# daigo0927/pwcnet

Measured on AMD Instinct MI355X. Metric: image_pairs_per_sec_448x1024, higher is better.
Workload: dtype f32 via fp16x2-split MFMA (fp32 tensors and accumulation; big stride-1 convs, level-1 extractor and correlation on the F16 pipe)

## Files before the change

pwcnet_amd/_lib.py:

```python
import ctypes
import os
import subprocess

import torch

_HERE = os.path.dirname(os.path.abspath(__file__))
CSRC = os.path.join(_HERE, "csrc")
HARNESS = os.environ.get("PWC_HARNESS", "") == "1"
LIB_PATH = os.path.join(CSRC, "libpwc_hip_harness.so" if HARNESS else "libpwc_hip.so")
HARNESS_SIGNATURES_NAMES = ("pwc_debug_cost_volume_blk_rows", "pwc_debug_conv3x3_sk_tile", "pwc_debug_conv3x3_t32",
                            "pwc_debug_h2_reserve_cus")
SOURCES = ["conv3x3_mfma.hip", "conv3x3_wino.hip", "conv3x3_direct.hip", "cost_volume.hip", "pwc_ops.hip",
           "pwc_backward.hip", "conv3x3_wgrad.hip", "conv3x3_h2.hip", "conv3x3_c16pair.hip", "conv3x3_sk.hip", "conv3x3_t32.hip", "conv3x3_w32.hip",
           "pwc_flow_loss.hip", "pwc_unsup.hip", "pwc_census.hip", "pwc_fbcheck.hip"]
HEADERS = ["pwc_common.h", "conv_fp32_common.h", "cost_volume_common.h", "loss_common.h", "cost_volume_roll.hip", "cost_volume_mfma.hip", "cost_volume_h2.hip", "cost_volume_blk.hip", "conv3x3_wino4.hip", os.path.join("..", "..", "include", "pwc_hip.h")]

_vp, _i, _f, _l, _sz = ctypes.c_void_p, ctypes.c_int, ctypes.c_float, ctypes.c_long, ctypes.c_size_t

SIGNATURES = {
    "pwc_version": (_i, []),
    "pwc_error_string": (ctypes.c_char_p, [_i]),
    "pwc_cost_volume_f32": (_i, [_vp, _i, _vp, _i, _vp, _i, _i, _i, _i, _i, _i, _f, _vp]),
    "pwc_cost_volume_uses_rolling_kernel": (_i, [_i, _i, _i, _i, _i, _i, _i]),
    "pwc_warp_bilinear_f32": (_i, [_vp, _i, _vp, _i, _f, _vp, _i, _i, _i, _i, _i, _vp]),
    "pwc_warp_nearest_f32": (_i, [_vp, _i, _vp, _i, _f, _vp, _i, _i, _i, _i, _i, _vp]),
    "pwc_cost_volume_coarse_f32": (_i, [_vp, _i, _vp, _i, _vp, _i, _f, _vp, _i, _vp, _i, _i, _i, _i, _i, _i, _f, _vp]),
    "pwc_resize_bilinear_pair_f32": (_i, [_vp, _i, _vp, _i, _vp, _i, _vp, _i, _i, _i, _i, _i, _i, _i, _vp]),
    "pwc_warp_copy_f32": (_i, [_i, _vp, _i, _vp, _i, _f, _vp, _i, _i, _i, _i, _i, _vp, _i, _vp, _i, _i, _vp]),
    "pwc_warp_cost_volume_f32": (_i, [_vp, _i, _vp, _i, _vp, _i, _f, _vp, _i, _i, _i, _i, _i, _i, _f, _vp]),
    "pwc_warp_cost_volume_concat_f32": (_i, [_vp, _i, _vp, _i, _vp, _i, _f, _vp, _i, _i, _vp, _i, _i, _i, _i, _i, _i, _f, _vp]),
    "pwc_warp_cost_volume_concat_h2_f32": (_i, [_vp, _i, _vp, _i, _vp, _i, _f, _vp, _i, _i, _vp, _i, _i, _i, _i, _i, _i, _f, _vp]),
    "pwc_warp_cost_volume_concat_blk_f32": (_i, [_vp, _i, _vp, _i, _vp, _i, _f, _vp, _i, _i, _vp, _i, _i, _i, _i, _i, _i, _f, _vp]),
    "pwc_warp_cost_volume_concat_supported": (_i, [_i, _i, _i, _i, _i, _i, _i, _i, _i]),
    "pwc_warp_cost_volume_concat_blk_supported": (_i, [_i, _i, _i, _i, _i, _i, _i, _i, _i]),
    "pwc_conv3x3_packed_floats": (_sz, [_i, _i]),
    "pwc_conv3x3_pack_f32": (_i, [_vp, _vp, _i, _i, _i, _vp, _vp]),
    "pwc_conv3x3_f32": (_i, [_vp, _i, _vp, _vp, _vp, _i, _i, _i, _i, _i, _i, _i, _i, _i, _f, _i, _i, _vp, _sz, _vp]),
    "pwc_conv3x3_workspace_floats": (_sz, [_i, _i]),
    "pwc_conv3x3_plan": (_i, [_i, _i, _i, ctypes.POINTER(_i)]),
    "pwc_conv3x3_uses_halo_kernel": (_i, [_i, _i, _i, _i, _i]),
    "pwc_conv3x3_tile_shape": (_i, [_i, ctypes.POINTER(_i), ctypes.POINTER(_i)]),
    "pwc_conv3x3_wino_packed_floats": (_sz, [_i, _i]),
    "pwc_conv3x3_wino_pack_f32": (_i, [_vp, _vp, _i, _i, _i, _vp, _vp]),
    "pwc_conv3x3_wino_f32": (_i, [_vp, _i, _vp, _vp, _vp, _i, _i, _i, _i, _i, _i, _i, _i, _f, _vp]),
    "pwc_conv3x3_wino_workgroups": (_l, [_i, _i, _i, _i, _i]),
    "pwc_conv3x3_wino4_packed_floats": (_sz, [_i, _i]),
    "pwc_conv3x3_wino4_pack_f32": (_i, [_vp, _vp, _i, _i, _i, _vp, _vp]),
    "pwc_conv3x3_wino4_f32": (_i, [_vp, _i, _vp, _vp, _vp, _i, _i, _i, _i, _i, _i, _i, _i, _f, _vp]),
    "pwc_conv3x3_wino4_supported": (_i, [_i, _i, _i, _i, _i, _i]),
    "pwc_conv3x3_h2_packed_floats": (_sz, [_i, _i]),
    "pwc_conv3x3_h2_pack_f32": (_i, [_vp, _vp, _i, _i, _i, _vp, _vp]),
    "pwc_conv3x3_h2_f32": (_i, [_vp, _i, _vp, _vp, _vp, _i, _i, _i, _i, _i, _i, _i, _i, _f, _vp, _sz, _vp]),
    "pwc_conv3x3_h2_ex_f32": (_i, [_vp, _i, _i, _vp, _i, _vp, _vp, _vp, _i, _i, _i, _i, _i, _i, _i, _i, _f, _vp, _sz, _vp, _vp]),
    "pwc_conv3x3_h2_ex3_f32": (_i, [_vp, _i, _i, _vp, _i, _i, _vp, _i, _vp, _vp, _vp, _i, _i, _i, _i, _i, _i, _i, _f, _vp, _sz, _vp, _vp]),
    "pwc_conv3x3_h2_workspace_floats": (_sz, [_i, _i, _i, _i, _i, _i]),
    "pwc_conv3x3_h2_supported": (_i, [_i, _i, _i, _i, _i, _i]),
    "pwc_conv3x3_h2_plan": (_i, [_i, _i, _i, _i, _i, _i]),
    "pwc_conv3x3_h2_stride2_f32": (_i, [_vp, _i, _vp, _vp, _vp, _i, _i, _i, _i, _i, _i, _i, _f, _vp, _sz, _vp, _vp]),
    "pwc_conv3x3_h2_stride2_supported": (_i, [_i, _i, _i, _i, _i]),
    "pwc_conv3x3_sk_packed_floats": (_sz, [_i, _i]),
    "pwc_conv3x3_sk_pack_f32": (_i, [_vp, _vp, _i, _i, _i, _vp, _vp]),
    "pwc_conv3x3_sk_f32": (_i, [_vp, _i, _vp, _vp, _vp, _i, _i, _i, _i, _i, _i, _i, _i, _i, _f, _vp]),
    "pwc_conv3x3_sk_supported": (_i, [_i, _i, _i, _i, _i, _i, _i]),
    "pwc_conv3x3_sk_variant_f32": (_i, [_vp, _i, _vp, _vp, _vp, _i, _i, _i, _i, _i, _i, _i, _i, _i, _f, _i, _vp]),
    "pwc_conv3x3_t32_packed_floats": (_sz, [_i]),
    "pwc_conv3x3_t32_pack_f32": (_i, [_vp, _vp, _i, _i, _vp, _vp]),
    "pwc_conv3x3_t32_f32": (_i, [_vp, _i, _vp, _vp, _vp, _i, _i, _i, _i, _i, _i, _i, _i, _f, _vp]),
    "pwc_conv3x3_t32_supported": (_i, [_i, _i, _i, _i, _i, _i]),
    "pwc_conv3x3_w32_packed_floats": (_sz, [_i]),
    "pwc_conv3x3_w32_pack_f32": (_i, [_vp, _vp, _i, _i, _vp, _vp]),
    "pwc_conv3x3_w32_f32": (_i, [_vp, _i, _vp, _vp, _vp, _i, _i, _i, _i, _i, _i, _i, _f, _vp]),
    "pwc_conv3x3_w32_supported": (_i, [_i, _i, _i, _i, _i, _i, _i]),
    "pwc_conv3x3_h2_stride2_packed_floats": (_sz, [_i, _i]),
    "pwc_conv3x3_h2_stride2_pack_f32": (_i, [_vp, _vp, _i, _i, _i, _vp, _vp]),
    "pwc_conv3x3_h2_stride2_workspace_floats": (_sz, [_i, _i, _i, _i, _i]),
    "pwc_conv3x3_c16pair_packed_floats": (_sz, []),
    "pwc_conv3x3_c16pair_pack_f32": (_i, [_vp, _vp, _vp, _vp]),
    "pwc_conv3x3_c16pair_f32": (_i, [_vp, _i, _vp, _vp, _vp, _vp, _i, _i, _i, _i, _f, _vp]),
    "pwc_conv3x3_c16pair_supported": (_i, [_i, _i, _i]),
    "pwc_conv3x3_c3c16pair_packed_floats": (_sz, []),
    "pwc_conv3x3_c3c16pair_pack_f32": (_i, [_vp, _vp, _vp, _vp, _vp]),
    "pwc_conv3x3_c3c16pair_f32": (_i, [_vp, _i, _vp, _i, _vp, _vp, _vp, _vp, _vp, _i, _i, _i, _f, _vp]),
    "pwc_conv3x3_c3c16pair_supported": (_i, [_i, _i, _i]),
    "pwc_conv3x3_h2_variant_f32": (_i, [_vp, _i, _vp, _vp, _vp, _i, _i, _i, _i, _i, _i, _i, _i, _f, _i, _vp, _sz, _vp]),
    "pwc_conv3x3_wino_split_plan": (_i, [_i, _i, _i, _i, _i, _i]),
    "pwc_conv3x3_wino_split_workspace_floats": (_sz, [_i, _i, _i, _i, _i]),
    "pwc_conv3x3_wino_split_f32": (_i, [_vp, _i, _vp, _vp, _vp, _i, _i, _i, _i, _i, _i, _i, _i, _f, _i, _vp, _sz, _vp]),
    "pwc_conv3x3_direct_f32": (_i, [_vp, _i, _vp, _vp, _vp, _i, _vp, _i, _i, _i, _i, _i, _i, _i, _i, _i, _f, _vp]),
    "pwc_resize_bilinear_f32": (_i, [_vp, _i, _vp, _i, _i, _i, _i, _i, _i, _i, _f, _vp]),
    "pwc_resize_bilinear_status_f32": (_i, [_vp, _i, _vp, _i, _i, _i, _i, _i, _i, _i, _f, _vp, _vp]),
    "pwc_absmax_f32": (_i, [_vp, _i, _l, _i, _vp, _vp]),
    "pwc_copy_channels_f32": (_i, [_vp, _i, _vp, _i, _l, _i, _vp]),
    "pwc_device_spin": (_i, [ctypes.c_longlong, _vp]),
    "pwc_device_touch": (_i, [_vp, _vp]),
    "pwc_lrelu_grad_f32": (_i, [_vp, _i, _vp, _i, _l, _i, _f, _vp]),
    "pwc_add_f32": (_i, [_vp, _i, _vp, _i, _l, _i, _f, _i, _vp]),
# ... 123 lines not shown
```

pwcnet_amd/csrc/conv3x3_h2.hip:

```cpp
#pragma once
#include "pwc_common.h"
#include <type_traits>

typedef float pwc_f32x16 __attribute__((ext_vector_type(16)));

struct H2Args {
    const float* x;
    const void* wp;
    const float* bias;
    float* y;
    int x_cs, y_cs;
    int N, H, W;
    int Cin_phys, Cout;
    int apply_act;
    float slope;
    int tiles_x, tiles_y, ncb;
    int dil_y, dil_x;
    int ntiles;
    float* ws_partial;
    unsigned* dbg;
    int Ho, Wo;
    const float* x2;
    int x2_cs, nc16_a;
    const float* x3;
// ... 414 lines not shown
        tap(std::integral_constant<int, 2>{}, std::integral_constant<int, 1>{}, g, buf, more, false);
        H2_STAMP(11);
        tap(std::integral_constant<int, 2>{}, std::integral_constant<int, 2>{}, g, buf, more, false);
        H2_STAMP(12);
        const bool tile_end = c16 == nc16 - 1;
        if (tile_end || !more) {
            if (ABL & 2048) tk0 = __builtin_readcyclecounter();
            if (piece_c0 != 0) {
                finish(tcur, 1, 0);
            } else if (tile_end) {
                finish(tcur, 0, 0);
            } else {
                const long tile_end_g = (long)(g - c16) + nc16;
                int nother = 0;
                for (int w2 = lw + 1; w2 < G && (long)w2 * total / G < tile_end_g; ++w2) ++nother;
                finish(tcur, 0, nother);
            }
            drain = true;
            piece_c0 = 0;
            if (ABL & 2048) tk_fin += __builtin_readcyclecounter() - tk0;
        }
        step(tcur, c16);
        step(t1, c1);
        step(t2, c2);
    }
    if ((ABL & 2048) && a.dbg && lane == 0) {
        unsigned* o = a.dbg + (lw * 8 + wave) * 4;
        o[0] = (unsigned)(__builtin_readcyclecounter() - tk_start); o[1] = (unsigned)tk_wait; o[2] = (unsigned)tk_bar; o[3] = (unsigned)tk_fin;
    }
#undef H2_STAMP
}

__global__ void conv3x3_h2_pack_kernel(const float* __restrict__ w, const int32_t* __restrict__ cin_map, int Cin,
                                       int Cin_phys, int Cout, int nct, unsigned short* __restrict__ packed, int s2) {
    const size_t total = (size_t)(Cin_phys >> 4) * nct * 9 * 32 * 16;
    for (size_t idx = blockIdx.x * (size_t)blockDim.x + threadIdx.x; idx < total;
         idx += (size_t)gridDim.x * blockDim.x) {
        const int ch = (int)(idx & 15);
        size_t r = idx >> 4;
        const int i = (int)(r & 31);
        r >>= 5;
        const int tap = (int)(r % 9);
        r /= 9;
        const int ct = (int)(r % nct);
        const int c16 = (int)(r / nct);
        const int ncc = Cin_phys >> 6, par = s2 ? c16 / ncc : 0;
        const int cphys = s2 ? (c16 - par * ncc) * 16 + ch : c16 * 16 + ch;
        const int clog = cin_map ? cin_map[cphys] : (cphys < Cin ? cphys : -1);
        const int co = ct * 32 + i;
        int wtap = tap;
        if (s2) {
            const int R = tap / 3, DX = tap - 3 * R, dy = 2 * (R - 1) + (par >> 1), dx = 2 * (DX - 1) + (par & 1);
            wtap = (R >= 1 && DX >= 1 && dy <= 2 && dx <= 2) ? dy * 3 + dx : -1;
        }
        float u = 0.f;
        if (wtap >= 0 && clog >= 0 && clog < Cin && co < Cout) u = w[((size_t)wtap * Cin + clog) * Cout + co];
        _Float16 h, m;
        pwc_split1(u, h, m);
        const int tr = tap / 3, dx = tap - 3 * tr;
        unsigned short* base = packed + (((((size_t)c16 * 3 + tr) * nct + ct) * 3 + dx) * 4) * 256;
        base[(ch >> 3) * 256 + i * 8 + (ch & 7)] = __builtin_bit_cast(unsigned short, h);
        base[(2 + (ch >> 3)) * 256 + i * 8 + (ch & 7)] = __builtin_bit_cast(unsigned short, m);
    }
}

extern "C" size_t pwc_conv3x3_h2_packed_floats(int Cin_phys, int Cout) {
    if (Cin_phys <= 0 || Cout <= 0) return 0;
    return (size_t)(Cin_phys >> 4) * ((Cout + 31) / 32) * 9 * (H2_TAPB / 4);
}

extern "C" int pwc_conv3x3_h2_pack_f32(const float* w_hwio, const int32_t* cin_map, int Cin, int Cin_phys,
                                       int Cout, float* packed, pwc_stream_t stream) {
    if (!w_hwio || !packed || Cin <= 0 || Cout <= 0 || Cin_phys < Cin) return PWC_EINVAL;
    if (Cin_phys % 16) return PWC_EALIGN;
    const int nct = (Cout + 31) / 32;
    const size_t total = (size_t)(Cin_phys >> 4) * nct * 9 * 32 * 16;
    int blocks = (int)((total + 255) / 256);
    if (blocks > 4096) blocks = 4096;
    hipLaunchKernelGGL(conv3x3_h2_pack_kernel, dim3(blocks), dim3(256), 0, (hipStream_t)stream, w_hwio, cin_map,
                       Cin, Cin_phys, Cout, nct, reinterpret_cast<unsigned short*>(packed), 0);
    return pwc_launch_status();
}

extern "C" size_t pwc_conv3x3_h2_stride2_packed_floats(int Cin_phys, int Cout) {
    return pwc_conv3x3_h2_packed_floats(4 * Cin_phys, Cout);
}
extern "C" int pwc_conv3x3_h2_stride2_pack_f32(const float* w_hwio, const int32_t* cin_map, int Cin, int Cin_phys,
                                               int Cout, float* packed, pwc_stream_t stream) {
    if (!w_hwio || !packed || Cin <= 0 || Cout <= 0 || Cin_phys < Cin) return PWC_EINVAL;
    if (Cin_phys % 16) return PWC_EALIGN;
    const int nct = (Cout + 31) / 32;
    const size_t total = (size_t)(Cin_phys >> 2) * nct * 9 * 32 * 16;
    int blocks = (int)((total + 255) / 256);
    if (blocks > 4096) blocks = 4096;
    hipLaunchKernelGGL(conv3x3_h2_pack_kernel, dim3(blocks), dim3(256), 0, (hipStream_t)stream, w_hwio, cin_map,
                       Cin, 4 * Cin_phys, Cout, nct, reinterpret_cast<unsigned short*>(packed), 1);
    return pwc_launch_status();
}

struct H2Variant { int couts, rows, nm; };
static inline H2Variant h2_variant(int v) {
    switch (v) {
        case 1: return {128, 8, 12};
        case 2: return {64, 16, 12};
        case 3: return {96, 8, 9};
        case 4: return {32, 16, 6};
        default: return {64, 8, 6};
    }
}
struct H2Geo { int dy, dx, xs, hs, ws; };
static inline H2Geo h2_geometry(int H, int W, int d, int Cout) {
    H2Geo g = {d, d, 1, (H + d - 1) / d, (W + d - 1) / d};
    if (g.ws < 24 && d % 2 == 0 && (W + d / 2 - 1) / (d / 2) >= 24 && Cout % 64 == 0) {
        g.dx = d / 2; g.xs = 2; g.ws = (W + g.dx - 1) / g.dx;
    }
    return g;
}
static inline long h2_blocks(int v, int N, const H2Geo& g, int Cout) {
    const H2Variant t = h2_variant(v);
    return (long)N * g.dy * g.dx * ((g.ws + 31) / 32) * ((g.hs + t.rows - 1) / t.rows) * (Cout / t.couts);
}
static int h2_plan(int N, int H, int W, int Cin_phys, int Cout, int dilation, long* blocks_out) {
    if (N <= 0 || H <= 0 || W <= 0 || dilation < 1 || Cin_phys < 16 || (Cin_phys % 16) || Cout < 32 || (Cout % 32) || Cout > H2_MAX_COUT) return 0;
    const H2Geo geo = h2_geometry(H, W, dilation, Cout);
    int best = 0;
    double best_cost = 0.;
    long best_blocks = 0;
    const int order[5] = {1, 2, 3, 5, 4};
    for (int oi = 0; oi < 5; ++oi) {
        const int v = order[oi];
        const H2Variant t = h2_variant(v);
        if (Cout % t.couts) continue;
        if (geo.xs == 2 && t.rows != 8) continue;
        const long nb = h2_blocks(v, N, geo, Cout);
        if (nb >= (1L << 31)) continue;
        const double cost = (nb <= 256 ? 1.0 : (double)nb / 256.0) * (t.nm + 3.6);
        if (!best || cost < best_cost) { best = v; best_cost = cost; best_blocks = nb; }
    }
    if (blocks_out) *blocks_out = best_blocks;
    return best;
}

static inline bool h2_split_pays(long ntiles, int nc16, int cus) {
    if (ntiles > cus) return ntiles * nc16 >= (long)H2_MIN_STAGES * cus;
    return ntiles < cus && ntiles * nc16 >= (long)H2_MIN_STAGES * cus && 2L * nc16 * (cus - ntiles) >= 11L * cus;
}

#ifdef PWC_HARNESS
static int h2_reserve_cus = 0;
extern "C" void pwc_debug_h2_reserve_cus(int n) { h2_reserve_cus = n < 0 ? 0 : n; }
#else
constexpr int h2_reserve_cus = 0;
#endif

static int h2_cu_count() {
    const int cus = pwc_cu_count() - h2_reserve_cus;
    return cus > 0 ? cus : 1;
}

extern "C" int pwc_conv3x3_h2_supported(int N, int H, int W, int Cin_phys, int Cout, int dilation) {
    long nb = 0;
    if (!h2_plan(N, H, W, Cin_phys, Cout, dilation, &nb)) return 0;
    const H2Geo geo = h2_geometry(H, W, dilation, Cout);
    const int hs = geo.hs, ws = geo.ws;
    const bool filled = nb >= 192 || (nb >= 64 && h2_split_pays(nb, Cin_phys >> 4, h2_cu_count()));
    return hs >= 7 && ws >= 24 && filled && Cin_phys >= 32 ? 1 : 0;
}

#ifdef PWC_HARNESS
static unsigned* h2_debug_counters = nullptr;
#else
constexpr unsigned* h2_debug_counters = nullptr;
#endif

template <int CT, int PT, int WCG, int ABL, int XS = 1, bool S2 = false>
static int h2_launch(H2Args& a, int hs, int ws, float* workspace, size_t workspace_floats, hipStream_t stream) {
    typedef H2Cfg<CT, PT, WCG, XS> C;
    a.tiles_x = (ws + 31) / 32; a.tiles_y = (hs + C::TR - 1) / C::TR; a.ncb = a.Cout / (32 * C::NCT);
    const long nblk = (long)a.N * a.dil_y * a.dil_x * a.tiles_x * a.tiles_y * a.ncb;
    if (nblk * (a.Cin_phys >> 4) >= (1L << 31)) return PWC_ERANGE;
    a.ntiles = (int)nblk;
    const int cus = h2_cu_count();
    int grid = a.ntiles;
    a.ws_partial = nullptr;
    const size_t part = (size_t)C::NCT * 32 * C::TR * 32;
    if (workspace && h2_split_pays(a.ntiles, a.Cin_phys >> 4, cus) && workspace_floats >= (size_t)cus * part) {
        grid = cus;
        a.ws_partial = workspace;
    }
    pwc_allow_dynamic_lds<&conv3x3_h2_kernel<CT, PT, WCG, ABL, XS, S2>>(C::LDS);
    hipLaunchKernelGGL((conv3x3_h2_kernel<CT, PT, WCG, ABL, XS, S2>), dim3((unsigned)grid), dim3(512), C::LDS, stream, a);
    return pwc_launch_status();
}

template <int ABL = 0>
static int h2_run(const float* x, int x_cs, const float* packed_w, const float* bias, float* y, int y_cs, int N, int H, int W,
                  int Cin_phys, int Cout, int dilation, int apply_act, float slope, pwc_stream_t stream, int variant = 0,
                  float* workspace = nullptr, size_t workspace_floats = 0, int stride = 1, const float* x2 = nullptr, int x2_cs = 0,
                  int Cin_a_phys = 0, uint32_t* status = nullptr, const float* x3 = nullptr, int x3_cs = 0, int Cin_b_phys = 0) {
    if (!x || !packed_w || !bias || !y) return PWC_EINVAL;
    if (x3 && !x2) return PWC_EINVAL;
    const int slack = x3 ? 12 : 0;
    if (x2) {
        const int cb = x3 ? Cin_b_phys : Cin_phys - Cin_a_phys;
        if (Cin_a_phys <= 0 || Cin_a_phys >= Cin_phys || (Cin_a_phys % 16) || x_cs < Cin_a_phys - slack || x2_cs < cb - slack) return PWC_EINVAL;
        if ((x2_cs & 3) || !pwc_aligned16(x2)) return PWC_EALIGN;
        if ((long)H * W * x2_cs * 4 >= (long)PWC_OOB) return PWC_ERANGE;
    }
    if (x3) {
        const int cc = Cin_phys - Cin_a_phys - Cin_b_phys;
        if (Cin_b_phys <= 0 || (Cin_b_phys % 16) || cc <= 0 || x3_cs < cc - 12 || dilation != 1) return PWC_EINVAL;
        if ((x3_cs & 3) || !pwc_aligned16(x3)) return PWC_EALIGN;
        if ((long)H * W * x3_cs * 4 >= (long)PWC_OOB) return PWC_ERANGE;
    }
    if (reinterpret_cast<uintptr_t>(status) & 7u) return PWC_EALIGN;
    if (dilation < 1 || (stride != 1 && stride != 2)) return PWC_EINVAL;
    const bool shape_ok = !(Cin_phys % 16 || Cout % 32 || Cout > H2_MAX_COUT || (stride == 2 && (dilation != 1 || (H & 1) || (W & 1) || x2)));
    if (const int rc = pwc_conv_io_check(x, x_cs, x2 ? Cin_a_phys - slack : Cin_phys, y, y_cs, Cout, packed_w, bias, N, H, W, shape_ok)) return rc;
    if (!pwc_aligned16(workspace)) return PWC_EALIGN;
    if (((long)H * W + W + 2) * x_cs * 4 >= (long)PWC_OOB || (long)H * W * y_cs * 4 >= (long)PWC_OOB) return PWC_ERANGE;
    H2Args a;
    a.x = x; a.wp = packed_w; a.bias = bias; a.y = y; a.x_cs = x_cs; a.y_cs = y_cs;
    a.N = N; a.H = H; a.W = W; a.Cin_phys = Cin_phys; a.Cout = Cout; a.apply_act = apply_act; a.slope = slope;
    const bool s2 = stride == 2;
    a.Ho = s2 ? H / 2 : H; a.Wo = s2 ? W / 2 : W;
    if (s2) a.Cin_phys = 4 * Cin_phys;
    const H2Geo geo = h2_geometry(a.Ho, a.Wo, dilation, Cout);
    a.dil_y = geo.dy; a.dil_x = geo.dx;
    a.dbg = h2_debug_counters;
    a.x2 = x2; a.x2_cs = x2_cs; a.nc16_a = x2 ? Cin_a_phys >> 4 : a.Cin_phys >> 4; a.status = status;
    a.x3 = x3; a.x3_cs = x3_cs; a.nc16_b = x3 ? Cin_b_phys >> 4 : (a.Cin_phys >> 4) - a.nc16_a;
    const int hs = geo.hs, ws = geo.ws;
    if (variant == 0) variant = h2_plan(N, a.Ho, a.Wo, a.Cin_phys, Cout, dilation, nullptr);
    if (variant < 1 || variant > 5) return PWC_EUNSUPPORTED;
    if (Cout % h2_variant(variant).couts) return PWC_EUNSUPPORTED;
    if (s2) {
        switch (variant) {
            case 1: return h2_launch<2, 2, 2, ABL, 1, true>(a, hs, ws, workspace, workspace_floats, (hipStream_t)stream);
            case 2: return h2_launch<2, 2, 1, ABL, 1, true>(a, hs, ws, workspace, workspace_floats, (hipStream_t)stream);
            case 3: return h2_launch<3, 1, 1, ABL, 1, true>(a, hs, ws, workspace, workspace_floats, (hipStream_t)stream);
            case 4: return h2_launch<1, 2, 1, ABL, 1, true>(a, hs, ws, workspace, workspace_floats, (hipStream_t)stream);
            default: return h2_launch<1, 2, 2, ABL, 1, true>(a, hs, ws, workspace, workspace_floats, (hipStream_t)stream);
        }
    }
    if (geo.xs == 2) {
        switch (variant) {
            case 1: return h2_launch<2, 2, 2, ABL, 2>(a, hs, ws, workspace, workspace_floats, (hipStream_t)stream);
            case 3: return h2_launch<3, 1, 1, ABL, 2>(a, hs, ws, workspace, workspace_floats, (hipStream_t)stream);
            case 5: return h2_launch<1, 2, 2, ABL, 2>(a, hs, ws, workspace, workspace_floats, (hipStream_t)stream);
            default: return PWC_EUNSUPPORTED;
        }
    }
    switch (variant) {
        case 1: return h2_launch<2, 2, 2, ABL>(a, hs, ws, workspace, workspace_floats, (hipStream_t)stream);
        case 2: return h2_launch<2, 2, 1, ABL>(a, hs, ws, workspace, workspace_floats, (hipStream_t)stream);
        case 3: return h2_launch<3, 1, 1, ABL>(a, hs, ws, workspace, workspace_floats, (hipStream_t)stream);
        case 4: return h2_launch<1, 2, 1, ABL>(a, hs, ws, workspace, workspace_floats, (hipStream_t)stream);
        default: return h2_launch<1, 2, 2, ABL>(a, hs, ws, workspace, workspace_floats, (hipStream_t)stream);
    }
}

extern "C" size_t pwc_conv3x3_h2_workspace_floats(int N, int H, int W, int Cin_phys, int Cout, int dilation) {
    long nb = 0;
    const int v = h2_plan(N, H, W, Cin_phys, Cout, dilation, &nb);
    const int cus = h2_cu_count();
    if (!v || !h2_split_pays(nb, Cin_phys >> 4, cus)) return 0;
    const H2Variant t = h2_variant(v);
    return (size_t)cus * t.couts * t.rows * 32;
}

extern "C" int pwc_conv3x3_h2_f32(const float* x, int x_cs, const float* packed_w, const float* bias, float* y,
                                  int y_cs, int N, int H, int W, int Cin_phys, int Cout, int dilation,
                                  int apply_act, float slope, float* workspace, size_t workspace_floats, pwc_stream_t stream) {
    return h2_run<0>(x, x_cs, packed_w, bias, y, y_cs, N, H, W, Cin_phys, Cout, dilation, apply_act, slope, stream, 0,
                     workspace, workspace_floats);
}

extern "C" int pwc_conv3x3_h2_ex_f32(const float* x, int x_cs, int Cin_a_phys, const float* x2, int x2_cs,
                                     const float* packed_w, const float* bias, float* y, int y_cs, int N, int H, int W,
                                     int Cin_phys, int Cout, int dilation, int apply_act, float slope, float* workspace,
                                     size_t workspace_floats, uint32_t* status, pwc_stream_t stream) {
    return h2_run<0>(x, x_cs, packed_w, bias, y, y_cs, N, H, W, Cin_phys, Cout, dilation, apply_act, slope, stream, 0,
                     workspace, workspace_floats, 1, x2, x2_cs, Cin_a_phys, status);
}

extern "C" int pwc_conv3x3_h2_ex3_f32(const float* x, int x_cs, int Cin_a_phys, const float* x2, int x2_cs, int Cin_b_phys,
                                      const float* x3, int x3_cs, const float* packed_w, const float* bias, float* y, int y_cs,
                                      int N, int H, int W, int Cin_phys, int Cout, int apply_act, float slope, float* workspace,
                                      size_t workspace_floats, uint32_t* status, pwc_stream_t stream) {
    if (!x2 || !x3) return PWC_EINVAL;
    return h2_run<0>(x, x_cs, packed_w, bias, y, y_cs, N, H, W, Cin_phys, Cout, 1, apply_act, slope, stream, 0,
                     workspace, workspace_floats, 1, x2, x2_cs, Cin_a_phys, status, x3, x3_cs, Cin_b_phys);
}

extern "C" int pwc_conv3x3_h2_stride2_supported(int N, int H, int W, int Cin_phys, int Cout) {
    if (H <= 0 || W <= 0 || (H & 1) || (W & 1) || Cin_phys % 16 || Cin_phys > 32) return 0;
    return pwc_conv3x3_h2_supported(N, H / 2, W / 2, 4 * Cin_phys, Cout, 1);
}

extern "C" size_t pwc_conv3x3_h2_stride2_workspace_floats(int N, int H, int W, int Cin_phys, int Cout) {
    if ((H & 1) || (W & 1)) return 0;
    return pwc_conv3x3_h2_workspace_floats(N, H / 2, W / 2, 4 * Cin_phys, Cout, 1);
}

extern "C" int pwc_conv3x3_h2_stride2_f32(const float* x, int x_cs, const float* packed_w, const float* bias, float* y,
                                          int y_cs, int N, int H, int W, int Cin_phys, int Cout, int apply_act, float slope,
                                          float* workspace, size_t workspace_floats, uint32_t* status, pwc_stream_t stream) {
    return h2_run<0>(x, x_cs, packed_w, bias, y, y_cs, N, H, W, Cin_phys, Cout, 1, apply_act, slope, stream, 0,
                     workspace, workspace_floats, 2, nullptr, 0, 0, status);
}

extern "C" int pwc_conv3x3_h2_plan(int N, int H, int W, int Cin_phys, int Cout, int dilation) {
    return h2_plan(N, H, W, Cin_phys, Cout, dilation, nullptr);
}

extern "C" int pwc_conv3x3_h2_variant_f32(const float* x, int x_cs, const float* packed_w, const float* bias, float* y,
                                          int y_cs, int N, int H, int W, int Cin_phys, int Cout, int dilation,
                                          int apply_act, float slope, int variant, float* workspace, size_t workspace_floats,
// ... 6 lines not shown
```

pwcnet_amd/csrc/conv3x3_sk.hip:

```cpp
#include "pwc_common.h"

typedef unsigned int sk_u32x4 __attribute__((ext_vector_type(4)));
#define SK_OOB 0x80000000u

struct SkArgs {
    const float* x;
    const float* wp;
    const float* bias;
    float* y;
    int x_cs, y_cs;
    int N, H, W, Ho, Wo;
    int Cin_phys, Cout;
    int stride, dil, pad_t, pad_l;
    int apply_act;
    float slope;
    int nbx, nby;
    int ntx;
    int nct;
    int cg;
    int nsteps;
};

struct SkTile { int ct, tx, by, n; };
__device__ __forceinline__ SkTile sk_tile(const SkArgs& a) {
// ... 226 lines not shown
                }
            }
        }
    }

    __syncthreads();
#pragma unroll
    for (int mt = 0; mt < MT; ++mt)
#pragma unroll
        for (int nt = 0; nt < NT; ++nt) {
            const f32x4 s = __builtin_elementwise_fma(xx[mt][nt], f32x4{1.f / 2048.f, 1.f / 2048.f, 1.f / 2048.f, 1.f / 2048.f},
                                                      hh[mt][nt]);
            float* p = part + ((wave * MT + mt) * NT + nt) * 256;
#pragma unroll
            for (int r = 0; r < 4; ++r) p[(4 * kq + r) * 16 + m] = s[r];
        }
    __syncthreads();
    for (int it = t; it < MT * NT * 64; it += 512) {
        const int tile = it >> 6, px = (it >> 2) & 15, q = it & 3;
        const int mt = tile / NT, nt = tile - mt * NT;
        const int co = (ct * NT + nt) * 16 + q * 4;
        f32x4 v = *reinterpret_cast<const f32x4*>(a.bias + co);
#pragma unroll
        for (int w = 0; w < 8; ++w) v += *reinterpret_cast<const f32x4*>(part + ((w * MT + mt) * NT + nt) * 256 + px * 16 + q * 4);
        if (a.apply_act) {
#pragma unroll
            for (int k = 0; k < 4; ++k) v[k] = pwc_lrelu(v[k], a.slope);
        }
        const int oy = 4 * by + (px >> 2), ox = 4 * (tx * MT + mt) + (px & 3);
        if (oy < a.Ho && ox < a.Wo)
            *reinterpret_cast<f32x4*>(a.y + ((size_t)(n * a.Ho + oy) * a.Wo + ox) * a.y_cs + co) = v;
    }
}

__global__ void conv3x3_sk_pack_kernel(const float* __restrict__ w, const int32_t* __restrict__ cin_map, int Cin, int Cin_phys,
                                       int Cout, _Float16* __restrict__ packed) {
    const int cg = Cin_phys >> 5, nsteps = 9 * cg;
    const size_t total = (size_t)(Cout >> 4) * nsteps * 512;
    for (size_t idx = blockIdx.x * (size_t)blockDim.x + threadIdx.x; idx < total; idx += (size_t)gridDim.x * blockDim.x) {
        const int e = (int)(idx & 7), lane = (int)((idx >> 3) & 63);
        size_t r = idx >> 9;
        const int s = (int)(r % nsteps);
        const int cb = (int)(r / nsteps);
        const int tap = s / cg, c32 = s - tap * cg;
        const int cphys = c32 * 32 + (lane >> 4) * 8 + e;
        const int co = cb * 16 + (lane & 15);
        const int clog = cin_map ? cin_map[cphys] : (cphys < Cin ? cphys : -1);
        float v = 0.f;
        if (clog >= 0 && clog < Cin) v = w[((size_t)tap * Cin + clog) * Cout + co];
        _Float16* dst = packed + ((size_t)(cb * nsteps + s) * 2) * 512 + lane * 8 + e;
        pwc_split1(v, dst[0], dst[512]);
    }
}

static bool sk_shape_ok(int N, int H, int W, int Cin_phys, int Cout, int stride, int dilation) {
    if (N <= 0 || H <= 0 || W <= 0 || Cin_phys <= 0 || Cout <= 0) return false;
    if (Cin_phys % 32 || Cout % 16 || stride < 1 || stride > 2 || dilation < 1) return false;
    return true;
}

extern "C" size_t pwc_conv3x3_sk_packed_floats(int Cin_phys, int Cout) {
    if (Cin_phys <= 0 || Cout <= 0 || Cin_phys % 32 || Cout % 16) return 0;
    return (size_t)9 * Cin_phys * Cout;
}

extern "C" int pwc_conv3x3_sk_pack_f32(const float* w_hwio, const int32_t* cin_map, int Cin, int Cin_phys, int Cout,
                                       float* packed_w, pwc_stream_t stream) {
    if (!w_hwio || !packed_w || Cin <= 0 || Cout <= 0 || Cin_phys < Cin) return PWC_EINVAL;
    if (Cin_phys % 32 || Cout % 16) return PWC_EUNSUPPORTED;
    if (!pwc_aligned16(packed_w)) return PWC_EALIGN;
    const size_t total = (size_t)9 * Cin_phys * Cout * 2;
    int blocks = (int)((total + 255) / 256);
    if (blocks > 4096) blocks = 4096;
    hipLaunchKernelGGL(conv3x3_sk_pack_kernel, dim3(blocks), dim3(256), 0, (hipStream_t)stream, w_hwio, cin_map, Cin, Cin_phys,
                       Cout, reinterpret_cast<_Float16*>(packed_w));
    return pwc_launch_status();
}

#define PWC_SK_MAX_MACS 100000000L
#define PWC_SK_THIN_MACS 32000000L
#define PWC_SK_LP_MAX_MACS 240000000L
#define PWC_SK_LP_MAX_PIXELS 8192L
#define PWC_SK_S2_MAX_MACS 200000000L
extern "C" int pwc_conv3x3_sk_supported(int N, int H, int W, int Cin_phys, int Cout, int stride, int dilation) {
    if (!sk_shape_ok(N, H, W, Cin_phys, Cout, stride, dilation)) return 0;
    int Ho, Wo, pt, pl;
    pwc_same_pad(H, stride, dilation, &Ho, &pt);
    pwc_same_pad(W, stride, dilation, &Wo, &pl);
    if (!pwc_fits_2g(N, H, W, Cin_phys)) return 0;
    const long M = (long)N * Ho * Wo, macs = M * Cin_phys * Cout;
    if (stride == 1 && dilation == 1 && Cin_phys >= 96 && Cin_phys <= 288 && M <= PWC_SK_LP_MAX_PIXELS && macs <= PWC_SK_LP_MAX_MACS)
        return 1;
    if (stride == 2 && dilation == 1 && Cin_phys >= 64 && Cin_phys <= 128 && macs <= PWC_SK_S2_MAX_MACS) return 1;
    if (macs > PWC_SK_MAX_MACS) return 0;
    return (M <= 4096 || stride == 2 || macs <= PWC_SK_THIN_MACS) ? 1 : 0;
}

template <int MT, int NT, int PB>
static int sk_launch(SkArgs a, hipStream_t s) {
    a.ntx = (a.nbx + MT - 1) / MT;
    a.nct = a.Cout / (16 * NT);
    const long wgs = (long)a.N * a.nby * a.ntx * a.nct;
    if (wgs >= (1L << 31)) return PWC_ERANGE;
    hipLaunchKernelGGL((conv3x3_sk_kernel<MT, NT, PB>), dim3((unsigned)wgs), dim3(512), 0, s, a);
    return pwc_launch_status();
}

template <int MT, int NT, int PB, int S>
static int skp_launch(SkArgs a, hipStream_t s) {
    a.ntx = (a.nbx + MT - 1) / MT;
    a.nct = a.Cout / (16 * NT);
    const long wgs = (long)a.N * a.nby * a.ntx * a.nct;
    if (wgs >= (1L << 31)) return PWC_ERANGE;
    constexpr int NPX = (3 * S + 3) * ((4 * MT - 1) * S + 3);
    size_t lds = (size_t)NPX * (a.Cin_phys * 4 + 16);
    if (lds < (size_t)8 * MT * NT * 1024) lds = (size_t)8 * MT * NT * 1024;
    pwc_allow_dynamic_lds<&conv3x3_skp_kernel<MT, NT, PB, S>>(NPX * ((S == 1 ? 288 : 128) * 4 + 16));
    hipLaunchKernelGGL((conv3x3_skp_kernel<MT, NT, PB, S>), dim3((unsigned)wgs), dim3(512), lds, s, a);
    return pwc_launch_status();
}

#ifdef PWC_HARNESS
static int sk_tile_override = 0;
extern "C" int pwc_debug_conv3x3_sk_tile(int tile) { sk_tile_override = tile; return 0; }
#endif

static int sk_run(const float* x, int x_cs, const float* packed_w, const float* bias, float* y, int y_cs,
                  int N, int H, int W, int Cin_phys, int Cout, int stride, int dilation, int apply_act,
                  float slope, int tile_req, pwc_stream_t stream) {
    if (stride < 1 || stride > 2 || dilation < 1) return PWC_EINVAL;
    const bool shape_ok = !(Cin_phys % 32 || Cout % 16);
    if (const int rc = pwc_conv_io_check(x, x_cs, Cin_phys, y, y_cs, Cout, packed_w, bias, N, H, W, shape_ok)) return rc;
    if (!pwc_fits_2g(N, H, W, x_cs)) return PWC_ERANGE;
    SkArgs a;
    a.x = x; a.wp = packed_w; a.bias = bias; a.y = y; a.x_cs = x_cs; a.y_cs = y_cs;
    a.N = N; a.H = H; a.W = W;
    pwc_same_pad(H, stride, dilation, &a.Ho, &a.pad_t);
    pwc_same_pad(W, stride, dilation, &a.Wo, &a.pad_l);
    a.Cin_phys = Cin_phys; a.Cout = Cout; a.stride = stride; a.dil = dilation;
    a.apply_act = apply_act; a.slope = slope;
    a.nbx = (a.Wo + 3) / 4; a.nby = (a.Ho + 3) / 4;
    a.cg = Cin_phys / 32; a.nsteps = 9 * a.cg;
    a.ntx = a.nct = 0;
    const long wgs11 = (long)N * a.nbx * a.nby * (Cout / 16);
    int tile = wgs11 <= 256 ? 11 : (wgs11 <= 1024 || (Cout % 32)) ? 21 : 22;
    const bool lp_ok = dilation == 1 && ((stride == 1 && Cin_phys <= 288) || (stride == 2 && Cin_phys <= 128));
    if (lp_ok && stride == 1 && (Cin_phys >= 192 || (Cin_phys >= 96 && wgs11 > 256)))
        tile = wgs11 <= 256 ? 31 : (wgs11 <= 640 || (Cout % 32)) ? 41 : 42;
    if (lp_ok && stride == 2 && Cin_phys >= 64 && wgs11 > 256) tile = (wgs11 <= 640 || (Cout % 32)) ? 41 : 42;
    if (tile_req) {
        if (tile_req != 11 && tile_req != 21 && tile_req != 22 && tile_req != 31 && tile_req != 41 && tile_req != 42) return PWC_EINVAL;
        if (((tile_req % 10) == 2 && Cout % 32) || (tile_req > 30 && !lp_ok)) return PWC_EUNSUPPORTED;
        tile = tile_req;
    }
#ifdef PWC_HARNESS
    else if (sk_tile_override && !((sk_tile_override % 10) == 2 && Cout % 32) && !(sk_tile_override > 30 && !lp_ok)) tile = sk_tile_override;
#endif
    hipStream_t s = (hipStream_t)stream;
    switch (tile) {
        case 11: return sk_launch<1, 1, 5>(a, s);
        case 21: return sk_launch<2, 1, 3>(a, s);
        case 22: return sk_launch<2, 2, 2>(a, s);
        case 31: return stride == 1 ? skp_launch<1, 1, 11, 1>(a, s) : skp_launch<1, 1, 11, 2>(a, s);
        case 41: return stride == 1 ? skp_launch<2, 1, 7, 1>(a, s) : skp_launch<2, 1, 7, 2>(a, s);
        default: return stride == 1 ? skp_launch<2, 2, 3, 1>(a, s) : skp_launch<2, 2, 3, 2>(a, s);
    }
}

extern "C" int pwc_conv3x3_sk_f32(const float* x, int x_cs, const float* packed_w, const float* bias, float* y, int y_cs,
                                  int N, int H, int W, int Cin_phys, int Cout, int stride, int dilation, int apply_act,
                                  float slope, pwc_stream_t stream) {
    return sk_run(x, x_cs, packed_w, bias, y, y_cs, N, H, W, Cin_phys, Cout, stride, dilation, apply_act, slope, 0, stream);
}

extern "C" int pwc_conv3x3_sk_variant_f32(const float* x, int x_cs, const float* packed_w, const float* bias, float* y, int y_cs,
                                          int N, int H, int W, int Cin_phys, int Cout, int stride, int dilation, int apply_act,
                                          float slope, int tile, pwc_stream_t stream) {
    if (tile == 0) return PWC_EINVAL;
    return sk_run(x, x_cs, packed_w, bias, y, y_cs, N, H, W, Cin_phys, Cout, stride, dilation, apply_act, slope, tile, stream);
}
```

pwcnet_amd/csrc/pwc_common.h:

```cpp
#pragma once
#include <hip/hip_runtime.h>
#include <stdint.h>

#include "../../include/pwc_hip.h"

typedef float f32x4 __attribute__((ext_vector_type(4)));
typedef float f32x2 __attribute__((ext_vector_type(2)));
typedef _Float16 pwc_f16x8 __attribute__((ext_vector_type(8)));
typedef _Float16 pwc_f16x4 __attribute__((ext_vector_type(4)));
typedef _Float16 pwc_f16x2 __attribute__((ext_vector_type(2)));

#define PWC_WAVE 64

static inline int pwc_launch_status() {
    hipError_t e = hipGetLastError();
    return e == hipSuccess ? PWC_OK : (int)e;
}

template <auto Kernel>
static inline void pwc_allow_dynamic_lds(int bytes) {
    static unsigned long long done[4] = {0, 0, 0, 0};
    int d = 0;
    if (hipGetDevice(&d) == hipSuccess && d >= 0 && d < 256) {
        const unsigned long long bit = 1ull << (d & 63);
// ... 68 lines not shown
    return v;
}

#ifndef PWC_FENCE_BARRIER
#define PWC_FENCE_BARRIER 1
#endif
__device__ __forceinline__ void pwc_lds_barrier_raw() { asm volatile("s_waitcnt lgkmcnt(0)\n\ts_barrier" ::: "memory"); }
__device__ __forceinline__ void pwc_lds_barrier() {
#if PWC_FENCE_BARRIER
    __builtin_amdgcn_fence(__ATOMIC_RELEASE, "workgroup", "local");
    __builtin_amdgcn_s_barrier();
    __builtin_amdgcn_fence(__ATOMIC_ACQUIRE, "workgroup", "local");
#else
    pwc_lds_barrier_raw();
#endif
}

#define PWC_WAIT_VM(n) __builtin_amdgcn_s_waitcnt(((n) & 15) | (((n) >> 4) << 14) | (7 << 4) | (15 << 8))

__device__ __forceinline__ float pwc_lrelu(float v, float slope) {
    return fmaxf(v, slope * v);
}
__device__ __forceinline__ f32x4 pwc_lrelu4(f32x4 v, float slope) {
    return f32x4{pwc_lrelu(v[0], slope), pwc_lrelu(v[1], slope), pwc_lrelu(v[2], slope), pwc_lrelu(v[3], slope)};
}
__device__ __forceinline__ f32x4 pwc_lrelu4_packed(f32x4 v, float slope) {
    const f32x4 sv = v * slope;
    return f32x4{fmaxf(v[0], sv[0]), fmaxf(v[1], sv[1]), fmaxf(v[2], sv[2]), fmaxf(v[3], sv[3])};
}

__device__ __forceinline__ int pwc_xcd_remap(int b, int nblocks) {
    const int q = nblocks >> 3, r = nblocks & 7;
    const int xcd = b & 7, k = b >> 3;
    const int base = xcd < r ? xcd * (q + 1) : r * (q + 1) + (xcd - r) * q;
    return base + k;
}

__device__ __forceinline__ void pwc_split2(const float x0, const float x1, unsigned& h_pair, unsigned& m_pair) {
    const f32x2 xs = {x0, x1};
    const pwc_f16x2 h2 = __builtin_convertvector(xs, pwc_f16x2);
    const f32x2 xm = xs * 2048.f;
    const unsigned hp = __builtin_bit_cast(unsigned, h2);
    const float neg = -2048.f;
    unsigned mp;
    asm("v_fma_mixlo_f16 %0, %1, %2, %3 op_sel_hi:[1,0,0]" : "=v"(mp) : "v"(hp), "s"(neg), "v"(xm[0]));
    asm("v_fma_mixhi_f16 %0, %1, %2, %3 op_sel:[1,0,0] op_sel_hi:[1,0,0]" : "+v"(mp) : "v"(hp), "s"(neg), "v"(xm[1]));
    h_pair = hp; m_pair = mp;
}
__device__ __forceinline__ void pwc_split4(const f32x4 x, pwc_f16x4& h, pwc_f16x4& m) {
    typedef unsigned u32x2 __attribute__((ext_vector_type(2)));
    u32x2 hp, mp;
    unsigned a, b;
    pwc_split2(x[0], x[1], a, b); hp[0] = a; mp[0] = b;
    pwc_split2(x[2], x[3], a, b); hp[1] = a; mp[1] = b;
    h = __builtin_bit_cast(pwc_f16x4, hp);
    m = __builtin_bit_cast(pwc_f16x4, mp);
}
__device__ __forceinline__ void pwc_split4(const float x0, const float x1, const float x2, const float x3, pwc_f16x4& h, pwc_f16x4& m) {
    pwc_split4(f32x4{x0, x1, x2, x3}, h, m);
}
__device__ __forceinline__ void pwc_split1(const float x, _Float16& h, _Float16& m) {
    h = (_Float16)x;
    m = (_Float16)__builtin_fmaf((float)h, -2048.f, x * 2048.f);
}

template <int COUT = 32>
__global__ void conv3x3_c32_pack_kernel(const float* __restrict__ w, const int32_t* __restrict__ cin_map, int Cin, int Cin_phys,
                                        _Float16* __restrict__ packed) {
    static_assert(COUT == 32, "the row operand of v_mfma_f32_32x32x16_f16");
    const int j16 = Cin_phys >> 4;
    const int total = 9 * j16 * 512;
    for (int idx = blockIdx.x * blockDim.x + threadIdx.x; idx < total; idx += gridDim.x * blockDim.x) {
        const int e = idx & 7, lane = (idx >> 3) & 63;
        const int r = idx >> 9;
        const int j = r % j16, tap = r / j16;
        const int cphys = j * 16 + (lane >> 5) * 8 + e, co = lane & (COUT - 1);
        const int clog = cin_map ? cin_map[cphys] : (cphys < Cin ? cphys : -1);
        float v = 0.f;
        if (clog >= 0 && clog < Cin) v = w[((size_t)tap * Cin + clog) * COUT + co];
        _Float16* dst = packed + (size_t)r * 1024 + lane * 8 + e;
        pwc_split1(v, dst[0], dst[512]);
    }
}
```

Baseline: 3489.

## Add LDS-tiled stride-2 conv kernel with even/odd column split and route s2 convs

Adds a new stride-2 3x3 conv kernel. It stages a 4x32 output tile's input patch into LDS as fp16 hi/lo halves, with columns de-interleaved into even and odd halves, then runs 16x16x32 f16 MFMAs with double-buffered weight fetches. Stride-2 h2 layers with Cin_phys==32 and sk stride-2 layers with enough tiles are routed to it. The h2 stride-2 packed buffer grows to carry an extra sk-format weight image. The aim is to cut redundant input reads and raise MFMA use on the downsampling convs, at the cost of extra weight memory and new routing heuristics.

```diff
diff --git a/pwcnet_amd/_lib.py b/pwcnet_amd/_lib.py
--- a/pwcnet_amd/_lib.py
+++ b/pwcnet_amd/_lib.py
@@ -9,9 +9,9 @@
 HARNESS = os.environ.get("PWC_HARNESS", "") == "1"
 LIB_PATH = os.path.join(CSRC, "libpwc_hip_harness.so" if HARNESS else "libpwc_hip.so")
 HARNESS_SIGNATURES_NAMES = ("pwc_debug_cost_volume_blk_rows", "pwc_debug_conv3x3_sk_tile", "pwc_debug_conv3x3_t32",
-                            "pwc_debug_h2_reserve_cus")
+                            "pwc_debug_h2_reserve_cus", "pwc_debug_conv3x3_s2_tile")
 SOURCES = ["conv3x3_mfma.hip", "conv3x3_wino.hip", "conv3x3_direct.hip", "cost_volume.hip", "pwc_ops.hip",
-           "pwc_backward.hip", "conv3x3_wgrad.hip", "conv3x3_h2.hip", "conv3x3_c16pair.hip", "conv3x3_sk.hip", "conv3x3_t32.hip", "conv3x3_w32.hip",
+           "pwc_backward.hip", "conv3x3_wgrad.hip", "conv3x3_h2.hip", "conv3x3_c16pair.hip", "conv3x3_sk.hip", "conv3x3_s2.hip", "conv3x3_t32.hip", "conv3x3_w32.hip",
            "pwc_flow_loss.hip", "pwc_unsup.hip", "pwc_census.hip", "pwc_fbcheck.hip"]
 HEADERS = ["pwc_common.h", "conv_fp32_common.h", "cost_volume_common.h", "loss_common.h", "cost_volume_roll.hip", "cost_volume_mfma.hip", "cost_volume_h2.hip", "cost_volume_blk.hip", "conv3x3_wino4.hip", os.path.join("..", "..", "include", "pwc_hip.h")]
 
diff --git a/pwcnet_amd/csrc/conv3x3_h2.hip b/pwcnet_amd/csrc/conv3x3_h2.hip
--- a/pwcnet_amd/csrc/conv3x3_h2.hip
+++ b/pwcnet_amd/csrc/conv3x3_h2.hip
@@ -520,8 +520,13 @@
     return pwc_launch_status();
 }
 
+static inline bool h2s2_has_tile_image(int Cin_phys, int Cout) { return Cin_phys > 0 && Cout > 0 && !(Cin_phys % 32) && !(Cout % 16); }
+static inline size_t h2s2_tile_image_offset(int Cin_phys, int Cout) {
+    return (pwc_conv3x3_h2_packed_floats(4 * Cin_phys, Cout) + 3) & ~(size_t)3;
+}
 extern "C" size_t pwc_conv3x3_h2_stride2_packed_floats(int Cin_phys, int Cout) {
-    return pwc_conv3x3_h2_packed_floats(4 * Cin_phys, Cout);
+    if (!h2s2_has_tile_image(Cin_phys, Cout)) return pwc_conv3x3_h2_packed_floats(4 * Cin_phys, Cout);
+    return h2s2_tile_image_offset(Cin_phys, Cout) + pwc_conv3x3_sk_packed_floats(Cin_phys, Cout);
 }
 extern "C" int pwc_conv3x3_h2_stride2_pack_f32(const float* w_hwio, const int32_t* cin_map, int Cin, int Cin_phys,
                                                int Cout, float* packed, pwc_stream_t stream) {
@@ -533,7 +538,9 @@
     if (blocks > 4096) blocks = 4096;
     hipLaunchKernelGGL(conv3x3_h2_pack_kernel, dim3(blocks), dim3(256), 0, (hipStream_t)stream, w_hwio, cin_map,
                        Cin, 4 * Cin_phys, Cout, nct, reinterpret_cast<unsigned short*>(packed), 1);
-    return pwc_launch_status();
+    if (const int rc = pwc_launch_status()) return rc;
+    if (!h2s2_has_tile_image(Cin_phys, Cout)) return PWC_OK;
+    return pwc_conv3x3_sk_pack_f32(w_hwio, cin_map, Cin, Cin_phys, Cout, packed + h2s2_tile_image_offset(Cin_phys, Cout), stream);
 }
 
 struct H2Variant { int couts, rows, nm; };
@@ -629,6 +636,14 @@
     pwc_allow_dynamic_lds<&conv3x3_h2_kernel<CT, PT, WCG, ABL, XS, S2>>(C::LDS);
     hipLaunchKernelGGL((conv3x3_h2_kernel<CT, PT, WCG, ABL, XS, S2>), dim3((unsigned)grid), dim3(512), C::LDS, stream, a);
     return pwc_launch_status();
+}
+
+static bool h2s2_tile_routed(int N, int H, int W, int x_cs, int Cin_phys, int Cout) {
+    const bool ok = h2s2_has_tile_image(Cin_phys, Cout) && pwc_conv3x3_s2_tile_admits(N, H, W, x_cs, Cin_phys, Cout);
+#ifdef PWC_HARNESS
+    if (pwc_conv3x3_s2_tile_debug_mode()) return ok && pwc_conv3x3_s2_tile_debug_mode() > 0;
+#endif
+    return ok && Cin_phys == 32;
 }
 
 template <int ABL = 0>
@@ -672,6 +687,9 @@
     if (variant == 0) variant = h2_plan(N, a.Ho, a.Wo, a.Cin_phys, Cout, dilation, nullptr);
     if (variant < 1 || variant > 5) return PWC_EUNSUPPORTED;
     if (Cout % h2_variant(variant).couts) return PWC_EUNSUPPORTED;
+    if (s2 && h2s2_tile_routed(N, H, W, x_cs, Cin_phys, Cout))
+        return pwc_conv3x3_s2_tile_launch(x, x_cs, packed_w + h2s2_tile_image_offset(Cin_phys, Cout), bias, y, y_cs, N, H, W, Cin_phys,
+                                          Cout, apply_act, slope, stream);
     if (s2) {
         switch (variant) {
             case 1: return h2_launch<2, 2, 2, ABL, 1, true>(a, hs, ws, workspace, workspace_floats, (hipStream_t)stream);
diff --git a/pwcnet_amd/csrc/conv3x3_s2.hip b/pwcnet_amd/csrc/conv3x3_s2.hip
--- /dev/null
+++ b/pwcnet_amd/csrc/conv3x3_s2.hip
@@ -0,0 +1,203 @@
+#include "pwc_common.h"
+
+typedef unsigned int s2_u32x4 __attribute__((ext_vector_type(4)));
+#define S2_OOB 0x80000000u
+
+constexpr int S2_PC = 2 * PWC_S2_TILE_COLS + 1;
+constexpr int S2_PR = 2 * PWC_S2_TILE_ROWS + 1;
+constexpr int S2_NPX = S2_PR * S2_PC;
+constexpr int S2_EVEN = PWC_S2_TILE_COLS + 1;
+constexpr int S2_LINE = S2_PC * 32;
+constexpr int S2_CC = 64;
+constexpr int S2_UB = 5;
+
+struct S2Args {
+    const float* x;
+    const float* wp;
+    const float* bias;
+    float* y;
+    int x_cs, y_cs;
+    int N, H, W, Ho, Wo;
+    int Cin_phys, Cout;
+    int pad_t, pad_l;
+    int apply_act;
+    float slope;
+    int ntx, nty;
+    int cg;
+    int nsteps;
+};
+
+template <int NBW>
+__global__ __launch_bounds__(512) void conv3x3_s2_kernel(const S2Args a) {
+    extern __shared__ __attribute__((aligned(16))) char s2_smem[];
+    const int t = threadIdx.x, lane = t & 63;
+    const int wave = __builtin_amdgcn_readfirstlane(t >> 6);
+    int b = blockIdx.x;
+    const int tx = b % a.ntx;
+    b /= a.ntx;
+    const int ty = b % a.nty, n = b / a.nty;
+
+    const __amdgpu_buffer_rsrc_t rx = __builtin_amdgcn_make_buffer_rsrc(
+        (void*)a.x, 0, (int)((size_t)a.N * a.H * a.W * a.x_cs * 4), 0x00020000);
+    const __amdgpu_buffer_rsrc_t rw = __builtin_amdgcn_make_buffer_rsrc(
+        (void*)a.wp, 0, (int)((size_t)a.Cout * a.nsteps * 128), 0x00020000);
+    const int m = lane & 15, kq = lane >> 4;
+    const int row = wave >> 1, cb0 = (wave & 1) * NBW, nb = a.Cout >> 4;
+
+    f32x4 hh[2][NBW], xx[2][NBW];
+#pragma unroll
+    for (int hf = 0; hf < 2; ++hf)
+#pragma unroll
+        for (int j = 0; j < NBW; ++j) {
+            hh[hf][j] = f32x4{0.f, 0.f, 0.f, 0.f};
+            xx[hf][j] = f32x4{0.f, 0.f, 0.f, 0.f};
+        }
+
+    auto fetch_b = [&](s2_u32x4 (&bv)[NBW][2], int s, bool live) {
+#pragma unroll
+        for (int j = 0; j < NBW; ++j) {
+            const int cb = cb0 + j;
+            const unsigned vo = (live && cb < nb) ? (unsigned)((cb * a.nsteps + s) * 2048 + lane * 16) : S2_OOB;
+            bv[j][0] = __builtin_amdgcn_raw_buffer_load_b128(rw, (int)vo, 0, 0);
+            bv[j][1] = __builtin_amdgcn_raw_buffer_load_b128(rw, (int)vo, 1024, 0);
+        }
+    };
+
+    const int gy0 = 2 * PWC_S2_TILE_ROWS * ty - a.pad_t, gx0 = 2 * PWC_S2_TILE_COLS * tx - a.pad_l;
+    for (int c0 = 0; c0 < a.Cin_phys; c0 += S2_CC) {
+        const int cc = a.Cin_phys - c0 < S2_CC ? a.Cin_phys - c0 : S2_CC;
+        const int cgc = cc >> 5, ng16 = cc >> 4, cqs = 1 + cgc;
+        const int nst = 9 * cgc, sbase = c0 >> 5;
+        auto gstep = [&](int si) { const int tap = si / cgc; return tap * a.cg + sbase + (si - tap * cgc); };
+        if (c0) __syncthreads();
+        s2_u32x4 b0[NBW][2], b1[NBW][2];
+        fetch_b(b0, gstep(0), true);
+        const int nu = S2_NPX << cqs;
+#pragma unroll 1
+        for (int u0 = t; u0 < nu; u0 += 512 * S2_UB) {
+            f32x4 v[S2_UB][2];
+            int dst[S2_UB];
+#pragma unroll
+            for (int k = 0; k < S2_UB; ++k) {
+                const int u = u0 + 512 * k;
+                const int px = u >> cqs, j = u - (px << cqs);
+                const int pr = px / S2_PC, pc = px - pr * S2_PC;
+                const int gy = gy0 + pr, gx = gx0 + pc;
+                const bool ok = u < nu && (unsigned)gy < (unsigned)a.H && (unsigned)gx < (unsigned)a.W;
+                const unsigned vo = ok ? (unsigned)(((n * a.H + gy) * a.W + gx) * a.x_cs + c0 + j * 8) * 4u : S2_OOB;
+                v[k][0] = __builtin_bit_cast(f32x4, __builtin_amdgcn_raw_buffer_load_b128(rx, (int)vo, 0, 0));
+                v[k][1] = __builtin_bit_cast(f32x4, __builtin_amdgcn_raw_buffer_load_b128(rx, (int)vo, 16, 0));
+                const int pos = (pc & 1) ? S2_EVEN + (pc >> 1) : pc >> 1;
+                dst[k] = u < nu ? ((pr * ng16 + (j >> 1)) * 2) * S2_LINE + pos * 32 + (j & 1) * 16 : -1;
+            }
+#pragma unroll
+            for (int k = 0; k < S2_UB; ++k)
+                if (dst[k] >= 0) {
+                    pwc_f16x4 h0, m0, h1, m1;
+                    pwc_split4(v[k][0], h0, m0);
+                    pwc_split4(v[k][1], h1, m1);
+                    *reinterpret_cast<pwc_f16x8*>(s2_smem + dst[k]) = __builtin_shufflevector(h0, h1, 0, 1, 2, 3, 4, 5, 6, 7);
+                    *reinterpret_cast<pwc_f16x8*>(s2_smem + dst[k] + S2_LINE) = __builtin_shufflevector(m0, m1, 0, 1, 2, 3, 4, 5, 6, 7);
+                }
+        }
+        __syncthreads();
+
+        auto step = [&](const s2_u32x4 (&bv)[NBW][2], int si) {
+            const int tap = si / cgc, c32 = si - tap * cgc;
+            const int dy = tap / 3, dx = tap - 3 * dy;
+            const int pos = (dx == 1 ? S2_EVEN : 0) + (dx >> 1) + m;
+            const char* p = s2_smem + (((2 * row + dy) * ng16 + 2 * c32 + (kq >> 1)) * 2) * S2_LINE + pos * 32 + (kq & 1) * 16;
+            pwc_f16x8 ah[2], am[2];
+#pragma unroll
+            for (int hf = 0; hf < 2; ++hf) {
+                ah[hf] = *reinterpret_cast<const pwc_f16x8*>(p + hf * 512);
+                am[hf] = *reinterpret_cast<const pwc_f16x8*>(p + hf * 512 + S2_LINE);
+            }
+#pragma unroll
+            for (int j = 0; j < NBW; ++j) {
+                const pwc_f16x8 wh = __builtin_bit_cast(pwc_f16x8, bv[j][0]);
+                const pwc_f16x8 wm = __builtin_bit_cast(pwc_f16x8, bv[j][1]);
+#pragma unroll
+                for (int hf = 0; hf < 2; ++hf) {
+                    xx[hf][j] = __builtin_amdgcn_mfma_f32_16x16x32_f16(wm, ah[hf], xx[hf][j], 0, 0, 0);
+                    hh[hf][j] = __builtin_amdgcn_mfma_f32_16x16x32_f16(wh, ah[hf], hh[hf][j], 0, 0, 0);
+                    xx[hf][j] = __builtin_amdgcn_mfma_f32_16x16x32_f16(wh, am[hf], xx[hf][j], 0, 0, 0);
+                }
+            }
+        };
+#pragma unroll 1
+        for (int si = 0; si < nst; si += 2) {
+            fetch_b(b1, gstep(si + 1 < nst ? si + 1 : 0), si + 1 < nst);
+            step(b0, si);
+            fetch_b(b0, gstep(si + 2 < nst ? si + 2 : 0), si + 2 < nst);
+            if (si + 1 < nst) step(b1, si + 1);
+        }
+    }
+
+    const int oy = PWC_S2_TILE_ROWS * ty + row;
+#pragma unroll
+    for (int hf = 0; hf < 2; ++hf) {
+        const int ox = PWC_S2_TILE_COLS * tx + hf * 16 + m;
+        if (oy < a.Ho && ox < a.Wo) {
+            float* yp = a.y + ((size_t)(n * a.Ho + oy) * a.Wo + ox) * a.y_cs + 4 * kq;
+#pragma unroll
+            for (int j = 0; j < NBW; ++j) {
+                const int cb = cb0 + j;
+                if (cb < nb) {
+                    f32x4 v = __builtin_elementwise_fma(xx[hf][j], f32x4{1.f / 2048.f, 1.f / 2048.f, 1.f / 2048.f, 1.f / 2048.f}, hh[hf][j]);
+                    v += *reinterpret_cast<const f32x4*>(a.bias + cb * 16 + 4 * kq);
+                    if (a.apply_act) v = pwc_lrelu4(v, a.slope);
+                    *reinterpret_cast<f32x4*>(yp + cb * 16) = v;
+                }
+            }
+        }
+    }
+}
+
+template <int NBW>
+static int s2_launch(const S2Args& a, hipStream_t s) {
+    const long wgs = (long)a.N * a.nty * a.ntx;
+    if (wgs >= (1L << 31)) return PWC_ERANGE;
+    const int cc = a.Cin_phys < S2_CC ? a.Cin_phys : S2_CC;
+    pwc_allow_dynamic_lds<&conv3x3_s2_kernel<NBW>>(S2_NPX * S2_CC * 4);
+    hipLaunchKernelGGL((conv3x3_s2_kernel<NBW>), dim3((unsigned)wgs), dim3(512), (size_t)S2_NPX * cc * 4, s, a);
+    return pwc_launch_status();
+}
+
+bool pwc_conv3x3_s2_tile_admits(int N, int H, int W, int x_cs, int Cin_phys, int Cout) {
+    if (N <= 0 || H <= 0 || W <= 0 || Cin_phys <= 0 || Cout <= 0 || x_cs < Cin_phys) return false;
+    if (Cin_phys % 32 || Cout % 16 || Cout > 128) return false;
+    return pwc_fits_2g(N, H, W, x_cs) && (long)Cout * 9 * (Cin_phys / 32) * 128 < (1L << 31);
+}
+
+long pwc_conv3x3_s2_tile_count(int N, int H, int W) {
+    const int Ho = (H + 1) / 2, Wo = (W + 1) / 2;
+    return (long)N * ((Ho + PWC_S2_TILE_ROWS - 1) / PWC_S2_TILE_ROWS) * ((Wo + PWC_S2_TILE_COLS - 1) / PWC_S2_TILE_COLS);
+}
+
+int pwc_conv3x3_s2_tile_launch(const float* x, int x_cs, const float* packed_w, const float* bias, float* y, int y_cs, int N, int H,
+                               int W, int Cin_phys, int Cout, int apply_act, float slope, pwc_stream_t stream) {
+    if (!pwc_conv3x3_s2_tile_admits(N, H, W, x_cs, Cin_phys, Cout)) return PWC_EUNSUPPORTED;
+    S2Args a;
+    a.x = x; a.wp = packed_w; a.bias = bias; a.y = y; a.x_cs = x_cs; a.y_cs = y_cs;
+    a.N = N; a.H = H; a.W = W;
+    pwc_same_pad(H, 2, 1, &a.Ho, &a.pad_t);
+    pwc_same_pad(W, 2, 1, &a.Wo, &a.pad_l);
+    a.Cin_phys = Cin_phys; a.Cout = Cout; a.apply_act = apply_act; a.slope = slope;
+    a.ntx = (a.Wo + PWC_S2_TILE_COLS - 1) / PWC_S2_TILE_COLS;
+    a.nty = (a.Ho + PWC_S2_TILE_ROWS - 1) / PWC_S2_TILE_ROWS;
+    a.cg = Cin_phys / 32; a.nsteps = 9 * a.cg;
+    hipStream_t s = (hipStream_t)stream;
+    switch ((Cout / 16 + 1) / 2) {
+        case 1: return s2_launch<1>(a, s);
+        case 2: return s2_launch<2>(a, s);
+        case 3: return s2_launch<3>(a, s);
+        default: return s2_launch<4>(a, s);
+    }
+}
+
+#ifdef PWC_HARNESS
+static int s2_tile_mode = 0;
+extern "C" int pwc_debug_conv3x3_s2_tile(int mode) { s2_tile_mode = mode; return 0; }
+int pwc_conv3x3_s2_tile_debug_mode() { return s2_tile_mode; }
+#endif
diff --git a/pwcnet_amd/csrc/conv3x3_sk.hip b/pwcnet_amd/csrc/conv3x3_sk.hip
--- a/pwcnet_amd/csrc/conv3x3_sk.hip
+++ b/pwcnet_amd/csrc/conv3x3_sk.hip
@@ -332,6 +332,7 @@
 #define PWC_SK_LP_MAX_MACS 240000000L
 #define PWC_SK_LP_MAX_PIXELS 8192L
 #define PWC_SK_S2_MAX_MACS 200000000L
+#define PWC_SK_S2_TILE_MIN 192L
 extern "C" int pwc_conv3x3_sk_supported(int N, int H, int W, int Cin_phys, int Cout, int stride, int dilation) {
     if (!sk_shape_ok(N, H, W, Cin_phys, Cout, stride, dilation)) return 0;
     int Ho, Wo, pt, pl;
@@ -398,6 +399,15 @@
     if (lp_ok && stride == 1 && (Cin_phys >= 192 || (Cin_phys >= 96 && wgs11 > 256)))
         tile = wgs11 <= 256 ? 31 : (wgs11 <= 640 || (Cout % 32)) ? 41 : 42;
     if (lp_ok && stride == 2 && Cin_phys >= 64 && wgs11 > 256) tile = (wgs11 <= 640 || (Cout % 32)) ? 41 : 42;
+    const bool s2_ok = stride == 2 && dilation == 1 && pwc_conv3x3_s2_tile_admits(N, H, W, x_cs, Cin_phys, Cout);
+    bool s2_tile = tile_req == 50 || (!tile_req && s2_ok && pwc_conv3x3_s2_tile_count(N, H, W) >= PWC_SK_S2_TILE_MIN);
+#ifdef PWC_HARNESS
+    if (!tile_req && pwc_conv3x3_s2_tile_debug_mode()) s2_tile = s2_ok && pwc_conv3x3_s2_tile_debug_mode() > 0;
+#endif
+    if (s2_tile) {
+        if (!s2_ok) return PWC_EUNSUPPORTED;
+        return pwc_conv3x3_s2_tile_launch(x, x_cs, packed_w, bias, y, y_cs, N, H, W, Cin_phys, Cout, apply_act, slope, stream);
+    }
     if (tile_req) {
         if (tile_req != 11 && tile_req != 21 && tile_req != 22 && tile_req != 31 && tile_req != 41 && tile_req != 42) return PWC_EINVAL;
         if (((tile_req % 10) == 2 && Cout % 32) || (tile_req > 30 && !lp_ok)) return PWC_EUNSUPPORTED;
diff --git a/pwcnet_amd/csrc/pwc_common.h b/pwcnet_amd/csrc/pwc_common.h
--- a/pwcnet_amd/csrc/pwc_common.h
+++ b/pwcnet_amd/csrc/pwc_common.h
@@ -174,3 +174,13 @@
         pwc_split1(v, dst[0], dst[512]);
     }
 }
+
+#define PWC_S2_TILE_ROWS 4
+#define PWC_S2_TILE_COLS 32
+bool pwc_conv3x3_s2_tile_admits(int N, int H, int W, int x_cs, int Cin_phys, int Cout);
+long pwc_conv3x3_s2_tile_count(int N, int H, int W);
+int pwc_conv3x3_s2_tile_launch(const float* x, int x_cs, const float* packed_w, const float* bias, float* y, int y_cs, int N, int H,
+                               int W, int Cin_phys, int Cout, int apply_act, float slope, pwc_stream_t stream);
+#ifdef PWC_HARNESS
+int pwc_conv3x3_s2_tile_debug_mode();
+#endif
```

After: 3531 (median of 6 runs). +1.2%, better.
